# jmoraispk/DeepMIMO

Hardware: AMD Instinct MI355X
Metric: user-channels/sec (higher is better)
Workload: dtype f16x3-split MFMA, f32 accumulate

## Files before the change

### deepmimo_amd/csrc/k2_channel_fd_fold.hip

```cpp
#include "dmx_common.h"
#include "dmx_tuning.h"

namespace dmx {

typedef _Float16 fh8 __attribute__((ext_vector_type(8)));
typedef _Float16 fh2 __attribute__((ext_vector_type(2)));
typedef __fp16 fhp2 __attribute__((ext_vector_type(2)));
typedef float ff16 __attribute__((ext_vector_type(16)));
typedef unsigned fu4 __attribute__((ext_vector_type(4)));

static constexpr int FOLD_TROW = 272;
static constexpr float FOLD_B_SCALE = 64.0f;
static constexpr int FOLD_MAX_M = 128;
static constexpr int FOLD_SHARED_FROM = 33;
static constexpr size_t FOLD_MIN_LDS = 160 * 1024 / 5 + 64;

struct FoldArgs {
    int64_t user_begin;
    int m_tx, ue_mh, bs_mh;
    int M, K;
    int sc_first, sc_stride;
    double inv_n;
    int ch;
    int sch;
    int nblk;
    int nchunk;
    int nsuper;
    int nb_last;
    int tab_rows;
    int adaptive;
    int k_tail;
    int mlog;
};

typedef float fv2 __attribute__((ext_vector_type(2)));

__device__ __forceinline__ void fold_split2(float x0, float x1, fh2& hi, fh2& lo, float m1) {
    const fhp2 h = __builtin_amdgcn_cvt_pkrtz(x0, x1);
    const fh2 hh = __builtin_bit_cast(fh2, h);
    const float r0 = __builtin_fmaf((float)hh[0], m1, x0);
    const float r1 = __builtin_fmaf((float)hh[1], m1, x1);
    const fhp2 l = __builtin_amdgcn_cvt_pkrtz(r0, r1);
    hi = hh;
    lo = __builtin_bit_cast(fh2, l);
}

__device__ __forceinline__ unsigned fold_bits(float x) { return __builtin_bit_cast(unsigned, x); }

__device__ __forceinline__ float fold_max_paths(float v) {
    int x = __builtin_bit_cast(int, v);
    v = fmaxf(v, __builtin_bit_cast(float, __builtin_amdgcn_update_dpp(x, x, 0xB1, 0xF, 0xF, false)));
    x = __builtin_bit_cast(int, v);
    v = fmaxf(v, __builtin_bit_cast(float, __builtin_amdgcn_update_dpp(x, x, 0x4E, 0xF, 0xF, false)));
    x = __builtin_bit_cast(int, v);
    v = fmaxf(v, __builtin_bit_cast(float, __builtin_amdgcn_update_dpp(x, x, 0x141, 0xF, 0xF, false)));
    x = __builtin_bit_cast(int, v);
    v = fmaxf(v, __builtin_bit_cast(float, __builtin_amdgcn_update_dpp(x, x, 0x140, 0xF, 0xF, false)));
    x = __builtin_bit_cast(int, v);
    return fmaxf(__builtin_bit_cast(float, __builtin_amdgcn_readlane(x, 0)), __builtin_bit_cast(float, __builtin_amdgcn_readlane(x, 16)));
}

__device__ __forceinline__ void wave_lds_sync() {
    __builtin_amdgcn_fence(__ATOMIC_ACQ_REL, "workgroup");
    __builtin_amdgcn_wave_barrier();
}

__host__ __device__ inline size_t fold_static_bytes(int tab_rows, int M) { return (size_t)tab_rows * 12 + align_up((size_t)M * 4, 16); }
__host__ __device__ inline size_t fold_wave_bytes(int M, int ch) { return 256 + (size_t)(M + ch) * FOLD_TROW; }

template <int WS>
__device__ __forceinline__ void fold_sync() {
    if constexpr (WS == 4) __syncthreads();
    else wave_lds_sync();
}


typedef float ff4 __attribute__((ext_vector_type(4)));
struct FoldX { ff4 x0, x1, y0, y1; };
#define FOLD_X_IO(X) "+{v[112:115]}"((X).x0), "+{v[116:119]}"((X).x1), "+{v[120:123]}"((X).y0), "+{v[124:127]}"((X).y1)

__device__ __forceinline__ uint32_t fold_lds_addr(const void* p) {
    return (uint32_t)(size_t)(__attribute__((address_space(3))) const void*)p;
}

__device__ __forceinline__ void fold_load0(FoldX& X, uint32_t ar, uint32_t er) {
    asm volatile(
        "ds_read_b128 v[112:115], %4\n\t"
        "ds_read_b128 v[116:119], %4 offset:16\n\t"
        "ds_read_b128 v[120:123], %5\n\t"
        "ds_read_b128 v[124:127], %5 offset:16"
        : "={v[112:115]}"(X.x0), "={v[116:119]}"(X.x1), "={v[120:123]}"(X.y0), "={v[124:127]}"(X.y1)
        : "v"(ar), "v"(er));
}

__device__ __forceinline__ void fold_drain(FoldX& X) { asm volatile("s_waitcnt lgkmcnt(0)" : FOLD_X_IO(X)); }

#define FOLD_CMUL_TEXT                                                                                               \
    "s_waitcnt lgkmcnt(0)\n\t"                                                                                       \
    "v_pk_mul_f32 v[108:109], v[112:113], v[120:121] op_sel:[1,1] op_sel_hi:[1,0]\n\t"                                \
    "v_pk_mul_f32 v[110:111], v[114:115], v[122:123] op_sel:[1,1] op_sel_hi:[1,0]\n\t"                                \
    "v_pk_fma_f32 v[112:113], v[112:113], v[120:121], v[108:109] op_sel_hi:[0,1,1] neg_lo:[0,0,1]\n\t"                \
    "v_pk_fma_f32 v[114:115], v[114:115], v[122:123], v[110:111] op_sel_hi:[0,1,1] neg_lo:[0,0,1]\n\t"                \
    "v_pk_mul_f32 v[108:109], v[116:117], v[124:125] op_sel:[1,1] op_sel_hi:[1,0]\n\t"                                \
    "v_pk_mul_f32 v[110:111], v[118:119], v[126:127] op_sel:[1,1] op_sel_hi:[1,0]\n\t"                                \
    "v_pk_fma_f32 v[116:117], v[116:117], v[124:125], v[108:109] op_sel_hi:[0,1,1] neg_lo:[0,0,1]\n\t"                \
    "v_pk_fma_f32 v[118:119], v[118:119], v[126:127], v[110:111] op_sel_hi:[0,1,1] neg_lo:[0,0,1]\n\t"
#define FOLD_CVT_HI_TEXT                                                                                             \
    "v_cvt_pkrtz_f16_f32 %0, v112, v113\n\t"                                                                         \
    "v_cvt_pkrtz_f16_f32 %1, v114, v115\n\t"                                                                         \
    "v_cvt_pkrtz_f16_f32 %2, v116, v117\n\t"                                                                         \
    "v_cvt_pkrtz_f16_f32 %3, v118, v119\n\t"
template <bool LO, int OFF>
__device__ __forceinline__ void fold_kstep(FoldX& X, float m1, uint32_t ar, uint32_t er, fh8& Ah, fh8& Al) {
    unsigned h0, h1, h2, h3;
    if constexpr (LO) {
        unsigned l0, l1, l2, l3;
        asm volatile(
            FOLD_CMUL_TEXT
            FOLD_CVT_HI_TEXT
            "v_fma_mix_f32 v112, %0, %14, v112 op_sel_hi:[1,0,0]\n\t"
            "v_fma_mix_f32 v113, %0, %14, v113 op_sel:[1,0,0] op_sel_hi:[1,0,0]\n\t"
            "v_fma_mix_f32 v114, %1, %14, v114 op_sel_hi:[1,0,0]\n\t"
            "v_fma_mix_f32 v115, %1, %14, v115 op_sel:[1,0,0] op_sel_hi:[1,0,0]\n\t"
            "v_fma_mix_f32 v116, %2, %14, v116 op_sel_hi:[1,0,0]\n\t"
            "v_fma_mix_f32 v117, %2, %14, v117 op_sel:[1,0,0] op_sel_hi:[1,0,0]\n\t"
            "v_fma_mix_f32 v118, %3, %14, v118 op_sel_hi:[1,0,0]\n\t"
            "v_fma_mix_f32 v119, %3, %14, v119 op_sel:[1,0,0] op_sel_hi:[1,0,0]\n\t"
            "v_cvt_pkrtz_f16_f32 %4, v112, v113\n\t"
            "v_cvt_pkrtz_f16_f32 %5, v114, v115\n\t"
            "v_cvt_pkrtz_f16_f32 %6, v116, v117\n\t"
            "v_cvt_pkrtz_f16_f32 %7, v118, v119\n\t"
            "ds_read_b128 v[112:115], %12 offset:%15\n\t"
            "ds_read_b128 v[116:119], %12 offset:%16\n\t"
            "ds_read_b128 v[120:123], %13 offset:%15\n\t"
            "ds_read_b128 v[124:127], %13 offset:%16"
            : "=&v"(h0), "=&v"(h1), "=&v"(h2), "=&v"(h3), "=&v"(l0), "=&v"(l1), "=&v"(l2), "=&v"(l3), FOLD_X_IO(X)
            : "v"(ar), "v"(er), "s"(m1), "i"(OFF), "i"(OFF + 16)
            : "v108", "v109", "v110", "v111");
        Al = __builtin_bit_cast(fh8, fu4{l0, l1, l2, l3});
    } else {
        asm volatile(
            FOLD_CMUL_TEXT
            FOLD_CVT_HI_TEXT
            "ds_read_b128 v[112:115], %8 offset:%10\n\t"
            "ds_read_b128 v[116:119], %8 offset:%11\n\t"
            "ds_read_b128 v[120:123], %9 offset:%10\n\t"
            "ds_read_b128 v[124:127], %9 offset:%11"
            : "=&v"(h0), "=&v"(h1), "=&v"(h2), "=&v"(h3), FOLD_X_IO(X)
            : "v"(ar), "v"(er), "i"(OFF), "i"(OFF + 16)
            : "v108", "v109", "v110", "v111");
    }
    Ah = __builtin_bit_cast(fh8, fu4{h0, h1, h2, h3});
    if constexpr (!LO) Al = Ah;
}
#undef FOLD_CMUL_TEXT
#undef FOLD_CVT_HI_TEXT

__device__ __forceinline__ uint32_t fold_rowbits_off(uint32_t r, int mlog, uint32_t K8) {
    return (r & ((1u << mlog) - 1u)) * K8 + ((r >> mlog) << 7);
}

template <int NS>
__device__ __forceinline__ void fold_finish(ff16& acc0, ff16& acc1, fv2 osc, fv2 (&w)[8]) {
    if constexpr (NS > 1) {
        asm volatile("s_nop 15" : "+v"(acc0), "+v"(acc1));
        fv2 t[8];
#pragma unroll
        for (int i = 0; i < 8; ++i) {
            const fv2 a = {acc0[2 * i], acc0[2 * i + 1]}, b = {acc1[2 * i], acc1[2 * i + 1]};
            asm volatile("v_pk_add_f32 %0, %1, %2" : "=v"(t[i]) : "v"(a), "v"(b));
        }
#pragma unroll
        for (int i = 0; i < 8; ++i) asm volatile("v_pk_mul_f32 %0, %1, %2" : "=v"(w[i]) : "v"(t[i]), "v"(osc));
    } else {
        asm volatile("s_nop 15" : "+v"(acc0));
#pragma unroll
        for (int i = 0; i < 8; ++i) {
            const fv2 a = {acc0[2 * i], acc0[2 * i + 1]};
            asm volatile("v_pk_mul_f32 %0, %1, %2" : "=v"(w[i]) : "v"(a), "v"(osc));
        }
    }
}

template <int S, int NS, bool LW>
__device__ __forceinline__ void fold_ksteps(FoldX& X, float m1, uint32_t ar, uint32_t er, uint32_t arn, uint32_t ern,
                                            ff16& acc0, ff16& acc1, const fh8 (&Bhi)[4], const fh8 (&Blo)[4]) {
    constexpr bool weak = LW && S == NS - 1;
    fh8 Ah, Al;
    if constexpr (S == NS - 1) fold_kstep<!weak, 0>(X, m1, arn, ern, Ah, Al);
    else fold_kstep<true, (S + 1) * 64>(X, m1, ar, er, Ah, Al);
    __builtin_amdgcn_sched_barrier(0);
    if constexpr (S & 1) {
        acc1 = __builtin_amdgcn_mfma_f32_32x32x16_f16(Ah, Bhi[S], acc1, 0, 0, 0);
        if constexpr (!weak) {
            acc1 = __builtin_amdgcn_mfma_f32_32x32x16_f16(Ah, Blo[S], acc1, 0, 0, 0);
            acc1 = __builtin_amdgcn_mfma_f32_32x32x16_f16(Al, Bhi[S], acc1, 0, 0, 0);
        }
    } else {
        acc0 = __builtin_amdgcn_mfma_f32_32x32x16_f16(Ah, Bhi[S], acc0, 0, 0, 0);
        if constexpr (!weak) {
            acc0 = __builtin_amdgcn_mfma_f32_32x32x16_f16(Ah, Blo[S], acc0, 0, 0, 0);
            acc0 = __builtin_amdgcn_mfma_f32_32x32x16_f16(Al, Bhi[S], acc0, 0, 0, 0);
        }
    }
    __builtin_amdgcn_sched_barrier(0);
    if constexpr (S + 1 < NS) fold_ksteps<S + 1, NS, LW>(X, m1, ar, er, arn, ern, acc0, acc1, Bhi, Blo);
}

struct FoldStoreCtx {
    __amdgpu_buffer_rsrc_t orsrc;
    uint32_t lane_col;
    uint32_t lane_row;
    uint32_t lmask_last;
    uint32_t K8;
    int mlog;
    int nb;
    int lane_hh;
    int tail_lane_dead;
    bool masked;
};

template <bool NT, int WS, int NS, bool LW, bool SROW>
__device__ __forceinline__ void fold_tiles(int sub, int ntiles, const uint32_t* rowsrc, const uint32_t* rowoff, int lp, int hh,
                                           const unsigned char* Ac, const unsigned char* E1, const fh8 (&Bhi)[4], const fh8 (&Blo)[4],
                                           float m1, fv2 osc, const FoldStoreCtx& c) {
    if (sub >= ntiles) return;
    constexpr int AUX = NT ? 2 : 0;
    const int rows = c.nb << (SROW ? c.mlog : 0);
    const int rt_chk = !SROW ? 0 : (c.masked ? (((c.nb - 1) << c.mlog) >> 5) : ((rows & 31) ? ntiles - 1 : ntiles));
    uint32_t P[4], D[4];
    if constexpr (SROW) {
#pragma unroll
        for (int q = 0; q < 4; ++q) { P[q] = fold_rowbits_off((uint32_t)q, c.mlog, c.K8); D[q] = fold_rowbits_off((uint32_t)(8 * q), c.mlog, c.K8); }
    }
    const uint32_t ac_lds = fold_lds_addr(Ac) + (uint32_t)hh * 32u, e1_lds = fold_lds_addr(E1) + (uint32_t)hh * 32u;
    uint32_t src = rowsrc[(sub << 5) + lp];
    uint32_t ar = ac_lds + (src >> 16), er = e1_lds + (src & 0xFFFFu);
    FoldX X;
    fold_load0(X, ar, er);
    for (int rt = sub; rt < ntiles; rt += WS) {
        const int rtn = rt + WS < ntiles ? rt + WS : rt;
        const uint32_t srcn = rowsrc[(rtn << 5) + lp];
        const uint32_t arn = ac_lds + (srcn >> 16), ern = e1_lds + (srcn & 0xFFFFu);
        ff16 acc0, acc1;
#pragma unroll
        for (int i = 0; i < 16; ++i) { acc0[i] = 0.f; acc1[i] = 0.f; }
        fold_ksteps<0, NS, LW>(X, m1, ar, er, arn, ern, acc0, acc1, Bhi, Blo);
        ar = arn; er = ern;
        fv2 w[8];
        fold_finish<NS>(acc0, acc1, osc, w);
        if constexpr (SROW) {
            const uint32_t T = fold_rowbits_off((uint32_t)rt << 5, c.mlog, c.K8);
            if (rt < rt_chk) {
#pragma unroll
                for (int i = 0; i < 16; ++i)
                    __builtin_amdgcn_raw_buffer_store_b32(fold_bits(w[i >> 1][i & 1]), c.orsrc, c.lane_row, T + P[i & 3] + D[i >> 2], AUX);
            } else {
#pragma unroll
                for (int i = 0; i < 16; ++i) {
                    const int a_blk = ((rt << 5) + (i & 3) + 8 * (i >> 2) + 4 * c.lane_hh) >> c.mlog;
                    const bool dead = a_blk >= c.nb || (c.masked && a_blk == c.nb - 1 && c.tail_lane_dead);
                    __builtin_amdgcn_raw_buffer_store_b32(fold_bits(w[i >> 1][i & 1]), c.orsrc, dead ? 0x80000000u : c.lane_row,
                                                          T + P[i & 3] + D[i >> 2], AUX);
                }
            }
        } else {
            const uint4* ro4 = reinterpret_cast<const uint4*>(rowoff + (rt << 5) + 4 * hh);
            if (c.masked) {
#pragma unroll
                for (int g = 0; g < 4; ++g) {
                    const uint4 ro = ro4[2 * g];
                    __builtin_amdgcn_raw_buffer_store_b32(fold_bits(w[2 * g][0]), c.orsrc, c.lane_col + (ro.x & c.lmask_last), 0, AUX);
                    __builtin_amdgcn_raw_buffer_store_b32(fold_bits(w[2 * g][1]), c.orsrc, c.lane_col + (ro.y & c.lmask_last), 0, AUX);
                    __builtin_amdgcn_raw_buffer_store_b32(fold_bits(w[2 * g + 1][0]), c.orsrc, c.lane_col + (ro.z & c.lmask_last), 0, AUX);
                    __builtin_amdgcn_raw_buffer_store_b32(fold_bits(w[2 * g + 1][1]), c.orsrc, c.lane_col + (ro.w & c.lmask_last), 0, AUX);
                }
            } else {
#pragma unroll
                for (int g = 0; g < 4; ++g) {
                    const uint4 ro = ro4[2 * g];
                    __builtin_amdgcn_raw_buffer_store_b32(fold_bits(w[2 * g][0]), c.orsrc, c.lane_col + ro.x, 0, AUX);
                    __builtin_amdgcn_raw_buffer_store_b32(fold_bits(w[2 * g][1]), c.orsrc, c.lane_col + ro.y, 0, AUX);
                    __builtin_amdgcn_raw_buffer_store_b32(fold_bits(w[2 * g + 1][0]), c.orsrc, c.lane_col + ro.z, 0, AUX);
                    __builtin_amdgcn_raw_buffer_store_b32(fold_bits(w[2 * g + 1][1]), c.orsrc, c.lane_col + ro.w, 0, AUX);
                }
            }
        }
    }
    fold_drain(X);
}

template <bool NT, int WS, bool SROW>
__device__ __forceinline__ void fold_tiles_kind(int tile_kind, int sub, int ntiles, const uint32_t* rowsrc, const uint32_t* rowoff, int lp, int hh,
                                                const unsigned char* Ac, const unsigned char* E1, const fh8 (&Bhi)[4], const fh8 (&Blo)[4],
                                                float m1, fv2 osc, const FoldStoreCtx& c) {
    switch (tile_kind) {
        case 2: fold_tiles<NT, WS, 1, false, SROW>(sub, ntiles, rowsrc, rowoff, lp, hh, Ac, E1, Bhi, Blo, m1, osc, c); break;
        case 4: fold_tiles<NT, WS, 2, false, SROW>(sub, ntiles, rowsrc, rowoff, lp, hh, Ac, E1, Bhi, Blo, m1, osc, c); break;
        case 5: fold_tiles<NT, WS, 2, true, SROW>(sub, ntiles, rowsrc, rowoff, lp, hh, Ac, E1, Bhi, Blo, m1, osc, c); break;
        case 6: fold_tiles<NT, WS, 3, false, SROW>(sub, ntiles, rowsrc, rowoff, lp, hh, Ac, E1, Bhi, Blo, m1, osc, c); break;
        case 7: fold_tiles<NT, WS, 3, true, SROW>(sub, ntiles, rowsrc, rowoff, lp, hh, Ac, E1, Bhi, Blo, m1, osc, c); break;
        case 8: fold_tiles<NT, WS, 4, false, SROW>(sub, ntiles, rowsrc, rowoff, lp, hh, Ac, E1, Bhi, Blo, m1, osc, c); break;
        default: fold_tiles<NT, WS, 4, true, SROW>(sub, ntiles, rowsrc, rowoff, lp, hh, Ac, E1, Bhi, Blo, m1, osc, c); break;
    }
}

template <bool NT, int WS>
__global__ __launch_bounds__(256, 4) void k2_fd_fold(WsView ws, FoldArgs a, float* __restrict__ out, int64_t items) {
    extern __shared__ __attribute__((aligned(16))) unsigned char smem[];
    uint32_t* rowoff0 = reinterpret_cast<uint32_t*>(smem);
    uint32_t* rowoff1 = rowoff0 + a.tab_rows;
    uint32_t* rowsrc = rowoff1 + a.tab_rows;
    uint32_t* pidx = rowsrc + a.tab_rows;
    const int tid = threadIdx.x, lane = tid & 63;
    const int wave = __builtin_amdgcn_readfirstlane(tid >> 6);
    unsigned char* wbase = smem + fold_static_bytes(a.tab_rows, a.M) + (WS == 1 ? (size_t)wave * fold_wave_bytes(a.M, a.ch) : (size_t)0);
    float2* qtab = reinterpret_cast<float2*>(wbase);
    unsigned char* Ac = wbase + 256;
    unsigned char* E1 = Ac + (size_t)a.M * FOLD_TROW;

    const int M = a.M, K = a.K;
    for (int r = tid; r < a.tab_rows; r += 256) {
        const int ab = r / M, p = r - ab * M;
        const uint32_t off = (uint32_t)(p * K + 16 * ab) * 8u;
        const int nb0 = a.nchunk > 1 ? a.ch : a.nb_last;
        rowoff0[r] = ab < nb0 ? off : 0xC0000000u;
        uint32_t o1 = ab < a.nb_last ? off : 0xC0000000u;
        if (ab == a.nb_last - 1 && a.k_tail < 16) o1 |= 0x80000000u;
        rowoff1[r] = o1;
        const bool any = ab < (a.ch > a.nb_last ? a.ch : a.nb_last);
        rowsrc[r] = any ? ((uint32_t)(ab * FOLD_TROW) | ((uint32_t)(p * FOLD_TROW) << 16)) : 0u;
    }
    for (int p = tid; p < M; p += 256) {
        const int rx = p / a.m_tx, tx = p - rx * a.m_tx;
        pidx[p] = (uint32_t)(rx % a.ue_mh) | ((uint32_t)(rx / a.ue_mh) << 8) | ((uint32_t)(tx % a.bs_mh) << 16) |
                  ((uint32_t)(tx / a.bs_mh) << 24);
    }
    __syncthreads();

    const int lp = lane & 31, hh = lane >> 5;
    const int col = lane & 31, bsc = col >> 1, cpart = col & 1;
    const int kb = a.sc_stride * bsc;
    const float kbl = (float)(kb & 4095), kbf = (float)kb, cq = 0.25f * (float)cpart;
    const uint32_t lane_col = (uint32_t)col * 4u;
    const uint32_t lmask_last = bsc < a.k_tail ? 0x7FFFFFFFu : 0xFFFFFFFFu;
    const size_t user_floats = (size_t)M * K * 2;

    constexpr int IW = 4 / WS;
    const int sub = WS == 4 ? wave : 0;
    for (int64_t item = (int64_t)blockIdx.x * IW + (WS == 1 ? wave : 0); item < items; item += (int64_t)gridDim.x * IW) {
        const int64_t ul = a.nsuper == 1 ? item : item / a.nsuper;
        const int sc = a.nsuper == 1 ? 0 : (int)(item - ul * a.nsuper);
        const int64_t u = a.user_begin + ul;
        const int b0 = sc * a.sch;
        const int bn = (a.nblk - b0) < a.sch ? (a.nblk - b0) : a.sch;
        int n_act = ws.n_keep[u];
        n_act = n_act < 32 ? n_act : 32;
        if (n_act == 0) {
            float* __restrict__ oz = out + (size_t)ul * user_floats + (size_t)b0 * 32;
            const int k0 = b0 * 16, k1 = (k0 + bn * 16) < K ? (k0 + bn * 16) : K;
            const int nfl = (k1 - k0) * 2;
            for (int p = sub; p < M; p += WS)
                for (int i = lane; i < nfl; i += 64) oz[(size_t)p * K * 2 + i] = 0.f;
            continue;
        }
        const size_t rb = (size_t)u * ws.P + lp;
        const bool ok = lp < n_act;
        const float cr = ok ? ws.c_re[rb] : 0.f, ci = ok ? ws.c_im[rb] : 0.f;
        const double q = ok ? (double)ws.dn[rb] * a.inv_n : 0.0;
        const double rxy = ok ? ws.rx_y[rb] : 0.0, rxz = ok ? ws.rx_z[rb] : 0.0;
        const double txy = ok ? ws.tx_y[rb] : 0.0, txz = ok ? ws.tx_z[rb] : 0.0;
        const float m = fold_max_paths(fmaxf(fabsf(cr), fabsf(ci)));
        bool last_weak = false;
        if (a.adaptive) {
            const int l0w = ((n_act - 1) >> 3) << 3;
            const float a2 = fmaf(cr, cr, ci * ci);
            const float m2 = fold_max_paths(a2), mw2 = fold_max_paths(lp >= l0w ? a2 : 0.f);
            last_weak = l0w >= 8 && mw2 * 4194304.0f <= m2;
        }
        int e;
        (void)frexpf(m, &e);
        const float gs = ldexpf(1.0f, 10 - e);
        const float oscale = ldexpf(1.0f, e - 10 - 6);
        const fv2 osc = {oscale, oscale};
        const double qh = rint(q * 4096.0) * (1.0 / 4096.0);
        const float qhf = (float)qh, qlf = (float)(q - qh);
        const float cgr = cr * gs, cgi = ci * gs;
        fold_sync<WS>();
        if (lane < 32 && sub == 0) qtab[lane] = make_float2(qhf, qlf);
        for (int p = 2 * sub + hh; p < M; p += 2 * WS) {
            const uint32_t ix = pidx[p];
            const double ph = (double)(ix & 255u) * rxy + (double)((ix >> 8) & 255u) * rxz +
                              (double)((ix >> 16) & 255u) * txy + (double)(ix >> 24) * txz;
            float s, c;
            sincos_rev(frac_rev(ph), s, c);
            *reinterpret_cast<float2*>(Ac + (size_t)p * FOLD_TROW + lp * 8) = make_float2(cgr * c - cgi * s, cgr * s + cgi * c);
        }
        fold_sync<WS>();

        const int nsteps = (n_act + 7) >> 3;
        const int tile_kind = __builtin_amdgcn_readfirstlane(2 * nsteps + (last_weak ? 1 : 0));
        fh8 Bhi[4], Blo[4];
#pragma unroll
        for (int s = 0; s < 4; ++s) {
            Bhi[s] = fh8{0, 0, 0, 0, 0, 0, 0, 0};
            Blo[s] = Bhi[s];
            if (s < nsteps) {
#pragma unroll
                for (int jj = 0; jj < 4; ++jj) {
                    const float2 qq = qtab[8 * s + 4 * hh + jj];
                    const float p1 = fmaf(qq.x, kbl, cq);
                    float sn, cs;
                    sincos_rev(fmaf(qq.y, kbf, p1 - rintf(p1)), sn, cs);
                    fh2 ph, pl;
                    fold_split2(cs * FOLD_B_SCALE, sn * FOLD_B_SCALE, ph, pl, ws.neg_one);
                    Bhi[s][2 * jj] = ph[0]; Bhi[s][2 * jj + 1] = ph[1];
                    Blo[s][2 * jj] = pl[0]; Blo[s][2 * jj + 1] = pl[1];
                }
            }
        }

        for (int c0 = 0; c0 < bn; c0 += a.ch) {
        const int a0 = b0 + c0;
        const int nb = (bn - c0) < a.ch ? (bn - c0) : a.ch;
        const bool last = a0 + nb == a.nblk;
        float* __restrict__ o = out + (size_t)ul * user_floats + (size_t)a0 * 32;
        fold_sync<WS>();
        {
            const int dsc = a.sc_stride * 32 * WS;
            const float pw = qhf * (float)(dsc & 4095);
            float ws_, wc_;
            sincos_rev(fmaf(qlf, (float)dsc, pw - rintf(pw)), ws_, wc_);
            const float wr = wc_, wi = -ws_;
            float er_ = 1.f, ei_ = 0.f;
            int it = 0;
            for (int ab = 2 * sub + hh; ab < nb; ab += 2 * WS, ++it) {
                if ((it & 7) == 0) {
                    const int sca = a.sc_first + a.sc_stride * 16 * (a0 + ab);
                    const float p1 = qhf * (float)(sca & 4095);
                    float s, c;
                    sincos_rev(fmaf(qlf, (float)sca, p1 - rintf(p1)), s, c);
                    er_ = c; ei_ = -s;
                } else {
                    const float t = fmaf(-ei_, wi, er_ * wr);
                    ei_ = fmaf(ei_, wr, er_ * wi);
                    er_ = t;
                }
                *reinterpret_cast<float2*>(E1 + (size_t)ab * FOLD_TROW + lp * 8) = make_float2(er_, ei_);
            }
        }
        fold_sync<WS>();

        const uint32_t* rowoff = last ? rowoff1 : rowoff0;
        const int rows = nb * M;
        const int ntiles = (rows + 31) >> 5;
        FoldStoreCtx sc_;
        sc_.orsrc = __builtin_amdgcn_make_buffer_rsrc(o, 0, (int)((unsigned)(user_floats - (size_t)a0 * 32) * 4u), 0x00020000);
        sc_.lane_col = lane_col;
        sc_.K8 = (uint32_t)K * 8u;
        sc_.mlog = a.mlog;
        sc_.lane_row = lane_col + (a.mlog >= 0 ? (uint32_t)hh * fold_rowbits_off(4u, a.mlog, (uint32_t)K * 8u) : 0u);
        sc_.lmask_last = lmask_last;
        sc_.nb = nb;
        sc_.lane_hh = hh;
        sc_.tail_lane_dead = bsc >= a.k_tail;
        sc_.masked = last && a.k_tail < 16;
        if (a.mlog >= 0) fold_tiles_kind<NT, WS, true>(tile_kind, sub, ntiles, rowsrc, rowoff, lp, hh, Ac, E1, Bhi, Blo, ws.neg_one, osc, sc_);
        else fold_tiles_kind<NT, WS, false>(tile_kind, sub, ntiles, rowsrc, rowoff, lp, hh, Ac, E1, Bhi, Blo, ws.neg_one, osc, sc_);
        }
    }
}

bool fd_fold_supported(const dmx_params& prm, const WsView& ws) {
    (void)ws;
    const int64_t M = (int64_t)prm.ue_shape[0] * prm.ue_shape[1] * prm.bs_shape[0] * prm.bs_shape[1];
    return prm.sc_stride > 0 && prm.n_selected >= 1 && M <= FOLD_MAX_M;
}

static constexpr int FOLD_SUPER = 64;
static int fold_chunk_blocks(int M, int nblk, int forced, int table_sets) {
    const int cand[3] = {32, 16, 8};
    if (forced > 0) return forced < nblk ? forced : nblk;
    for (int want = 4; want >= 2; --want) {
        for (int ch : cand) {
            const int c = ch < nblk ? ch : nblk;
            const int tab = (M * c + 31) / 32 * 32;
            const size_t smem = fold_static_bytes(tab, M) + table_sets * fold_wave_bytes(M, c);
            if (smem * want <= 160 * 1024) return c;
        }
    }
    return 8 < nblk ? 8 : nblk;
}

bool fd_fold_preferred(const dmx_params& prm, const WsView& ws) {
    const int64_t M = (int64_t)prm.ue_shape[0] * prm.ue_shape[1] * prm.bs_shape[0] * prm.bs_shape[1];
    const int K = prm.n_selected;
    if (!fd_fold_supported(prm, ws) || K < (M <= 16 ? 4 : 6)) return false;
    if (M <= 32) return true;
    if (M <= 48) return K <= 512;
    if (M <= 64) return K <= 256;
    if (M <= 96) return K <= 128;
    return K <= 64;
}

int launch_channels_fd_fold(const dmx_params& prm, const WsView& ws, int64_t user_begin, int64_t user_count, float2* out,
                            int chunk_blocks, hipStream_t stream) {
    if (user_count == 0 || prm.n_selected == 0) return DMX_OK;
    if (!fd_fold_supported(prm, ws)) {
        set_error("the folded kernel needs a uniformly spaced subcarrier selection (dmx_params.sc_stride > 0) and at most %d antenna pairs", FOLD_MAX_M);
        return DMX_ERR_SHAPE;
    }
    FoldArgs a;
    a.user_begin = user_begin;
    a.m_tx = prm.bs_shape[0] * prm.bs_shape[1];
    a.ue_mh = prm.ue_shape[0];
    a.bs_mh = prm.bs_shape[0];
    a.M = prm.ue_shape[0] * prm.ue_shape[1] * a.m_tx;
    a.K = prm.n_selected;
    a.sc_first = prm.sc_first;
    a.sc_stride = prm.sc_stride;
    a.inv_n = 1.0 / (double)prm.n_subcarriers;
    a.nblk = (a.K + 15) / 16;
    if (chunk_blocks <= 0) {
        chunk_blocks = tuning_int("DMX_FOLD_CHUNK", 0);
        if (chunk_blocks != 8 && chunk_blocks != 16 && chunk_blocks != 32) chunk_blocks = 0;
    }
    bool shared = a.M >= FOLD_SHARED_FROM;
    if (const int f = tuning_int("DMX_FOLD_SHARED", -1); f >= 0) shared = f == 1;
    const int sets = shared ? 1 : 4;
    a.ch = fold_chunk_blocks(a.M, a.nblk, chunk_blocks, sets);
    a.sch = (FOLD_SUPER / a.ch) * a.ch;
    if (a.sch > a.nblk) a.sch = (a.nblk + a.ch - 1) / a.ch * a.ch;
    a.nsuper = (a.nblk + a.sch - 1) / a.sch;
    a.nchunk = (a.nblk + a.ch - 1) / a.ch;
    a.nb_last = a.nblk - a.ch * (a.nchunk - 1);
    a.tab_rows = (a.M * a.ch + 31) / 32 * 32;
    a.k_tail = a.K - 16 * (a.nblk - 1);
    a.adaptive = (prm.flags & DMX_FLAG_ADAPTIVE_TERMS) ? 1 : 0;
    a.mlog = -1;
    for (int b = 0; b < 8; ++b) if (a.M == (1 << b)) a.mlog = b;
    if (tuning_int("DMX_FOLD_ROWTABLE", 0) == 1) a.mlog = -1;
    if ((size_t)a.M * (size_t)a.K * 8 >= (size_t)1 << 30) { set_error("%d x %d outputs per user are too many for the folded kernel", a.M, a.K); return DMX_ERR_SHAPE; }
    size_t smem = fold_static_bytes(a.tab_rows, a.M) + sets * fold_wave_bytes(a.M, a.ch);
    if (smem > 160 * 1024) { set_error("folded kernel tables of %zu bytes exceed LDS", smem); return DMX_ERR_SHAPE; }
    if (smem < FOLD_MIN_LDS) smem = FOLD_MIN_LDS;
    const int64_t items = user_count * a.nsuper;
    const auto kernel = shared ? k2_fd_fold<true, 4> : k2_fd_fold<true, 1>;
    int64_t grid = resident_workgroups(kernel, 256, smem);
    const int64_t need = shared ? items : (items + 3) / 4;
    if (grid > need) grid = need;
    return launch_dyn_lds(kernel, "k2_fd_fold", dim3((unsigned)grid), dim3(256), smem, smem, stream, ws, a, reinterpret_cast<float*>(out), items);
}

}
```

Before: 6.474 million.

## Pack hi/lo split of short last K-step into one MFMA and share B phasors

When the last K-step covers at most two active paths, the code duplicates those path columns in LDS and packs the A hi and lo halves into one fh8 operand, with B laid out to match. The final step then needs one MFMA instead of three. B-phasor generation is also changed so each lane computes half the sincos values and gets its partner's through a DPP swap and byte permutes. This adds duplicate LDS writes and extra permute work, and the packed B layout depends on subtle lane and sign conventions.

```diff
diff --git a/deepmimo_amd/csrc/k2_channel_fd_fold.hip b/deepmimo_amd/csrc/k2_channel_fd_fold.hip
--- a/deepmimo_amd/csrc/k2_channel_fd_fold.hip
+++ b/deepmimo_amd/csrc/k2_channel_fd_fold.hip
@@ -46,6 +46,23 @@
 }
 
 __device__ __forceinline__ unsigned fold_bits(float x) { return __builtin_bit_cast(unsigned, x); }
+
+__device__ __forceinline__ void fold_phasor(float2 qq, float kbl, float kbf, float cq, float m1, unsigned& hi, unsigned& lo) {
+    const float p1 = fmaf(qq.x, kbl, cq);
+    float sn, cs;
+    sincos_rev(fmaf(qq.y, kbf, p1 - rintf(p1)), sn, cs);
+    fh2 ph, pl;
+    fold_split2(cs * FOLD_B_SCALE, sn * FOLD_B_SCALE, ph, pl, m1);
+    hi = __builtin_bit_cast(unsigned, ph);
+    lo = __builtin_bit_cast(unsigned, pl);
+}
+
+static constexpr unsigned FOLD_SEL_OWN = 0x03020100u, FOLD_SEL_ROT = 0x05040706u;
+__device__ __forceinline__ void fold_pair_words(unsigned own, unsigned flip, unsigned sel0, unsigned sel1, unsigned& first, unsigned& second) {
+    const unsigned other = (unsigned)__builtin_amdgcn_update_dpp(0, (int)own, 0xB1, 0xF, 0xF, true) ^ flip;
+    first = __builtin_amdgcn_perm(other, own, sel0);
+    second = __builtin_amdgcn_perm(other, own, sel1);
+}
 
 __device__ __forceinline__ float fold_max_paths(float v) {
     int x = __builtin_bit_cast(int, v);
@@ -156,6 +173,37 @@
 #undef FOLD_CMUL_TEXT
 #undef FOLD_CVT_HI_TEXT
 
+__device__ __forceinline__ void fold_kstep_packed(FoldX& X, float m1, uint32_t arn, uint32_t ern, fh8& Ap) {
+    const uint64_t upper = 0xFFFFFFFF00000000ull;
+    unsigned w0, w1, w2, w3;
+    asm volatile(
+        "s_waitcnt lgkmcnt(0)\n\t"
+        "v_pk_mul_f32 v[108:109], v[112:113], v[120:121] op_sel:[1,1] op_sel_hi:[1,0]\n\t"
+        "v_pk_mul_f32 v[110:111], v[114:115], v[122:123] op_sel:[1,1] op_sel_hi:[1,0]\n\t"
+        "v_pk_fma_f32 v[112:113], v[112:113], v[120:121], v[108:109] op_sel_hi:[0,1,1] neg_lo:[0,0,1]\n\t"
+        "v_pk_fma_f32 v[114:115], v[114:115], v[122:123], v[110:111] op_sel_hi:[0,1,1] neg_lo:[0,0,1]\n\t"
+        "v_cvt_pkrtz_f16_f32 v108, v112, v113\n\t"
+        "v_cvt_pkrtz_f16_f32 v109, v114, v115\n\t"
+        "v_fma_mix_f32 v112, v108, %10, v112 op_sel_hi:[1,0,0]\n\t"
+        "v_fma_mix_f32 v113, v108, %10, v113 op_sel:[1,0,0] op_sel_hi:[1,0,0]\n\t"
+        "v_fma_mix_f32 v114, v109, %10, v114 op_sel_hi:[1,0,0]\n\t"
+        "v_fma_mix_f32 v115, v109, %10, v115 op_sel:[1,0,0] op_sel_hi:[1,0,0]\n\t"
+        "v_cvt_pkrtz_f16_f32 v110, v112, v113\n\t"
+        "v_cvt_pkrtz_f16_f32 v111, v114, v115\n\t"
+        "v_cndmask_b32_e64 %2, v108, 0, %11\n\t"
+        "v_cndmask_b32_e64 %3, v109, 0, %11\n\t"
+        "v_cndmask_b32_e64 %0, v108, v110, %11\n\t"
+        "v_cndmask_b32_e64 %1, v109, v111, %11\n\t"
+        "ds_read_b128 v[112:115], %8\n\t"
+        "ds_read_b128 v[116:119], %8 offset:16\n\t"
+        "ds_read_b128 v[120:123], %9\n\t"
+        "ds_read_b128 v[124:127], %9 offset:16"
+        : "=&v"(w0), "=&v"(w1), "=&v"(w2), "=&v"(w3), FOLD_X_IO(X)
+        : "v"(arn), "v"(ern), "s"(m1), "s"(upper)
+        : "v108", "v109", "v110", "v111");
+    Ap = __builtin_bit_cast(fh8, fu4{w0, w1, w2, w3});
+}
+
 __device__ __forceinline__ uint32_t fold_rowbits_off(uint32_t r, int mlog, uint32_t K8) {
     return (r & ((1u << mlog) - 1u)) * K8 + ((r >> mlog) << 7);
 }
@@ -182,12 +230,15 @@
     }
 }
 
-template <int S, int NS, bool LW>
+template <int S, int NS, bool LW, bool PK>
 __device__ __forceinline__ void fold_ksteps(FoldX& X, float m1, uint32_t ar, uint32_t er, uint32_t arn, uint32_t ern,
                                             ff16& acc0, ff16& acc1, const fh8 (&Bhi)[4], const fh8 (&Blo)[4]) {
-    constexpr bool weak = LW && S == NS - 1;
+    static_assert(!(LW && PK), "the one-term rule wins over packing");
+    constexpr bool packed = PK && S == NS - 1;
+    constexpr bool weak = (LW || PK) && S == NS - 1;
     fh8 Ah, Al;
-    if constexpr (S == NS - 1) fold_kstep<!weak, 0>(X, m1, arn, ern, Ah, Al);
+    if constexpr (packed) { fold_kstep_packed(X, m1, arn, ern, Ah); Al = Ah; }
+    else if constexpr (S == NS - 1) fold_kstep<!weak, 0>(X, m1, arn, ern, Ah, Al);
     else fold_kstep<true, (S + 1) * 64>(X, m1, ar, er, Ah, Al);
     __builtin_amdgcn_sched_barrier(0);
     if constexpr (S & 1) {
@@ -204,7 +255,8 @@
         }
     }
     __builtin_amdgcn_sched_barrier(0);
-    if constexpr (S + 1 < NS) fold_ksteps<S + 1, NS, LW>(X, m1, ar, er, arn, ern, acc0, acc1, Bhi, Blo);
+    if constexpr (packed && NS == 1) asm volatile("" : : "v"(Ah));
+    if constexpr (S + 1 < NS) fold_ksteps<S + 1, NS, LW, PK>(X, m1, ar, er, arn, ern, acc0, acc1, Bhi, Blo);
 }
 
 struct FoldStoreCtx {
@@ -220,7 +272,7 @@
     bool masked;
 };
 
-template <bool NT, int WS, int NS, bool LW, bool SROW>
+template <bool NT, int WS, int NS, bool LW, bool SROW, bool PK = false>
 __device__ __forceinline__ void fold_tiles(int sub, int ntiles, const uint32_t* rowsrc, const uint32_t* rowoff, int lp, int hh,
                                            const unsigned char* Ac, const unsigned char* E1, const fh8 (&Bhi)[4], const fh8 (&Blo)[4],
                                            float m1, fv2 osc, const FoldStoreCtx& c) {
@@ -245,7 +297,7 @@
         ff16 acc0, acc1;
 #pragma unroll
         for (int i = 0; i < 16; ++i) { acc0[i] = 0.f; acc1[i] = 0.f; }
-        fold_ksteps<0, NS, LW>(X, m1, ar, er, arn, ern, acc0, acc1, Bhi, Blo);
+        fold_ksteps<0, NS, LW, PK>(X, m1, ar, er, arn, ern, acc0, acc1, Bhi, Blo);
         ar = arn; er = ern;
         fv2 w[8];
         fold_finish<NS>(acc0, acc1, osc, w);
@@ -301,6 +353,10 @@
         case 6: fold_tiles<NT, WS, 3, false, SROW>(sub, ntiles, rowsrc, rowoff, lp, hh, Ac, E1, Bhi, Blo, m1, osc, c); break;
         case 7: fold_tiles<NT, WS, 3, true, SROW>(sub, ntiles, rowsrc, rowoff, lp, hh, Ac, E1, Bhi, Blo, m1, osc, c); break;
         case 8: fold_tiles<NT, WS, 4, false, SROW>(sub, ntiles, rowsrc, rowoff, lp, hh, Ac, E1, Bhi, Blo, m1, osc, c); break;
+        case 10: fold_tiles<NT, WS, 1, false, SROW, true>(sub, ntiles, rowsrc, rowoff, lp, hh, Ac, E1, Bhi, Blo, m1, osc, c); break;
+        case 11: fold_tiles<NT, WS, 2, false, SROW, true>(sub, ntiles, rowsrc, rowoff, lp, hh, Ac, E1, Bhi, Blo, m1, osc, c); break;
+        case 12: fold_tiles<NT, WS, 3, false, SROW, true>(sub, ntiles, rowsrc, rowoff, lp, hh, Ac, E1, Bhi, Blo, m1, osc, c); break;
+        case 13: fold_tiles<NT, WS, 4, false, SROW, true>(sub, ntiles, rowsrc, rowoff, lp, hh, Ac, E1, Bhi, Blo, m1, osc, c); break;
         default: fold_tiles<NT, WS, 4, true, SROW>(sub, ntiles, rowsrc, rowoff, lp, hh, Ac, E1, Bhi, Blo, m1, osc, c); break;
     }
 }
@@ -340,8 +396,6 @@
 
     const int lp = lane & 31, hh = lane >> 5;
     const int col = lane & 31, bsc = col >> 1, cpart = col & 1;
-    const int kb = a.sc_stride * bsc;
-    const float kbl = (float)(kb & 4095), kbf = (float)kb, cq = 0.25f * (float)cpart;
     const uint32_t lane_col = (uint32_t)col * 4u;
     const uint32_t lmask_last = bsc < a.k_tail ? 0x7FFFFFFFu : 0xFFFFFFFFu;
     const size_t user_floats = (size_t)M * K * 2;
@@ -372,12 +426,14 @@
         const double txy = ok ? ws.tx_y[rb] : 0.0, txz = ok ? ws.tx_z[rb] : 0.0;
         const float m = fold_max_paths(fmaxf(fabsf(cr), fabsf(ci)));
         bool last_weak = false;
+        const int l0w = ((n_act - 1) >> 3) << 3;
         if (a.adaptive) {
-            const int l0w = ((n_act - 1) >> 3) << 3;
             const float a2 = fmaf(cr, cr, ci * ci);
             const float m2 = fold_max_paths(a2), mw2 = fold_max_paths(lp >= l0w ? a2 : 0.f);
             last_weak = l0w >= 8 && mw2 * 4194304.0f <= m2;
         }
+        const bool pack = n_act - l0w <= 2 && !last_weak;
+        const bool dup = pack && (unsigned)(lp - l0w) < 2u;
         int e;
         (void)frexpf(m, &e);
         const float gs = ldexpf(1.0f, 10 - e);
@@ -388,34 +444,52 @@
         const float cgr = cr * gs, cgi = ci * gs;
         fold_sync<WS>();
         if (lane < 32 && sub == 0) qtab[lane] = make_float2(qhf, qlf);
+        if (dup && sub == 0 && (hh || lp != l0w)) qtab[lp + 4 * hh + (lp - l0w)] = make_float2(qhf, qlf);
         for (int p = 2 * sub + hh; p < M; p += 2 * WS) {
             const uint32_t ix = pidx[p];
             const double ph = (double)(ix & 255u) * rxy + (double)((ix >> 8) & 255u) * rxz +
                               (double)((ix >> 16) & 255u) * txy + (double)(ix >> 24) * txz;
             float s, c;
             sincos_rev(frac_rev(ph), s, c);
-            *reinterpret_cast<float2*>(Ac + (size_t)p * FOLD_TROW + lp * 8) = make_float2(cgr * c - cgi * s, cgr * s + cgi * c);
+            const float2 v = make_float2(cgr * c - cgi * s, cgr * s + cgi * c);
+            *reinterpret_cast<float2*>(Ac + (size_t)p * FOLD_TROW + lp * 8) = v;
+            if (dup) *reinterpret_cast<float2*>(Ac + (size_t)p * FOLD_TROW + lp * 8 + 32) = v;
         }
         fold_sync<WS>();
 
         const int nsteps = (n_act + 7) >> 3;
-        const int tile_kind = __builtin_amdgcn_readfirstlane(2 * nsteps + (last_weak ? 1 : 0));
+        int tile_kind = __builtin_amdgcn_readfirstlane(2 * nsteps + (last_weak ? 1 : 0));
+        if (__builtin_amdgcn_readfirstlane(pack ? 1 : 0)) tile_kind = 9 + nsteps;
+        int lo_ = lane;
+        asm volatile("" : "+v"(lo_));
+        const int cpi = lo_ & 1, kb = a.sc_stride * ((lo_ >> 1) & 15);
+        const float2* qlane = qtab + 4 * hh + 2 * cpart;
+        const float kbl = (float)(kb & 4095), kbf = (float)kb, cq = 0.25f * (float)cpi;
+        const unsigned pflip = cpi ? 0x80000000u : 0x00008000u;
+        const unsigned psel0 = cpi ? FOLD_SEL_ROT : FOLD_SEL_OWN, psel1 = cpi ? FOLD_SEL_OWN : FOLD_SEL_ROT;
         fh8 Bhi[4], Blo[4];
 #pragma unroll
         for (int s = 0; s < 4; ++s) {
             Bhi[s] = fh8{0, 0, 0, 0, 0, 0, 0, 0};
             Blo[s] = Bhi[s];
             if (s < nsteps) {
-#pragma unroll
-                for (int jj = 0; jj < 4; ++jj) {
-                    const float2 qq = qtab[8 * s + 4 * hh + jj];
-                    const float p1 = fmaf(qq.x, kbl, cq);
-                    float sn, cs;
-                    sincos_rev(fmaf(qq.y, kbf, p1 - rintf(p1)), sn, cs);
-                    fh2 ph, pl;
-                    fold_split2(cs * FOLD_B_SCALE, sn * FOLD_B_SCALE, ph, pl, ws.neg_one);
-                    Bhi[s][2 * jj] = ph[0]; Bhi[s][2 * jj + 1] = ph[1];
-                    Blo[s][2 * jj] = pl[0]; Blo[s][2 * jj + 1] = pl[1];
+                if (pack && s == nsteps - 1) {
+                    unsigned h, l, h0, h1, l0, l1;
+                    fold_phasor(qlane[8 * s], kbl, kbf, cq, ws.neg_one, h, l);
+                    fold_pair_words(h, pflip, psel0, psel1, h0, h1);
+                    fold_pair_words(l, pflip, psel0, psel1, l0, l1);
+                    Bhi[s] = __builtin_bit_cast(fh8, fu4{h0, h1, hh ? 0u : l0, hh ? 0u : l1});
+                } else {
+                    unsigned h[2], l[2], wh[4], wl[4];
+#pragma unroll
+                    for (int t = 0; t < 2; ++t) fold_phasor(qlane[8 * s + t], kbl, kbf, cq, ws.neg_one, h[t], l[t]);
+#pragma unroll
+                    for (int t = 0; t < 2; ++t) {
+                        fold_pair_words(h[t], pflip, psel0, psel1, wh[t], wh[t + 2]);
+                        fold_pair_words(l[t], pflip, psel0, psel1, wl[t], wl[t + 2]);
+                    }
+                    Bhi[s] = __builtin_bit_cast(fh8, fu4{wh[0], wh[1], wh[2], wh[3]});
+                    Blo[s] = __builtin_bit_cast(fh8, fu4{wl[0], wl[1], wl[2], wl[3]});
                 }
             }
         }
@@ -447,6 +521,7 @@
                     er_ = t;
                 }
                 *reinterpret_cast<float2*>(E1 + (size_t)ab * FOLD_TROW + lp * 8) = make_float2(er_, ei_);
+                if (dup) *reinterpret_cast<float2*>(E1 + (size_t)ab * FOLD_TROW + lp * 8 + 32) = make_float2(er_, ei_);
             }
         }
         fold_sync<WS>();
```

Result: no change. 6.458 million (-0.3%).
